# Irish-77/adapting-2D-ViTs-for-3D-point-cloud-understanding

Measured on NVIDIA B200. Metric: tokenized clouds/sec (FPS+kNN+embed), higher is better.
Workload: dtype bf16

## Files before the change

adapting-2d-vits-for-3d-point-cloud-understanding_b200/csrc/knn.cu:

```cuda
#include <stdlib.h>

#include "common.cuh"

namespace p3tok {

constexpr int KNN_WARPS = 8;
constexpr int KNN_CPW = 4;
constexpr int KNN_TILE = 2048;
constexpr uint64_t KNN_SENTINEL = 0xffffffffffffffffull;

__device__ __forceinline__ uint64_t shfl_xor_u64(uint64_t v, int m) {
  uint32_t lo = (uint32_t)v, hi = (uint32_t)(v >> 32);
  lo = __shfl_xor_sync(0xffffffffu, lo, m);
  hi = __shfl_xor_sync(0xffffffffu, hi, m);
  return ((uint64_t)hi << 32) | lo;
}
__device__ __forceinline__ uint64_t shfl_u64(uint64_t v, int src) {
  uint32_t lo = (uint32_t)v, hi = (uint32_t)(v >> 32);
  lo = __shfl_sync(0xffffffffu, lo, src);
  hi = __shfl_sync(0xffffffffu, hi, src);
  return ((uint64_t)hi << 32) | lo;
}
__device__ __forceinline__ uint64_t umin64(uint64_t a, uint64_t b) { return a < b ? a : b; }
__device__ __forceinline__ uint64_t umax64(uint64_t a, uint64_t b) { return a < b ? b : a; }
// ... 164 lines not shown
  if (g0 >= G) return;
#pragma unroll
  for (int c = 0; c < KNN_CPW; ++c) {
    if (qn[c] > 0) (void)merge_queue(c, L[c], qn[c]);
    const int g = g0 + c;
    if (g >= G) continue;
    const size_t o = ((size_t)b * G + g) * k;
#pragma unroll
    for (int j = 0; j < KPL; ++j) {
      const int r = j * 32 + lane;
      if (r < k) {
        const uint32_t id = (uint32_t)L[c][j];
        if (idx_is_i64) reinterpret_cast<int64_t*>(idx_out)[o + r] = (int64_t)id;
        else reinterpret_cast<int32_t*>(idx_out)[o + r] = (int32_t)id;
        if (dist_out) dist_out[o + r] = ord2f((uint32_t)(L[c][j] >> 32));
      }
    }
  }
}

template <int KPL>
static int knn_launch(const float* x, int B, int N, int pt_stride, const float* centres, int G, int k,
                      int mode, void* idx_out, int i64, float* dist_out, cudaStream_t s) {
  dim3 grid((unsigned)((G + KNN_WARPS * KNN_CPW - 1) / (KNN_WARPS * KNN_CPW)), (unsigned)B);
  if (mode == P3TOK_KNN_APF_SQ)
    knn_kernel<KPL, P3TOK_KNN_APF_SQ><<<grid, KNN_WARPS * 32, 0, s>>>(x, N, pt_stride, centres, G, k, idx_out, i64, dist_out);
  else
    knn_kernel<KPL, P3TOK_KNN_P4P_CDIST><<<grid, KNN_WARPS * 32, 0, s>>>(x, N, pt_stride, centres, G, k, idx_out, i64, dist_out);
  P3_LAUNCH_CHECK("knn_kernel");
  return P3TOK_OK;
}


#ifndef KNS_MIN_BLOCKS
#define KNS_MIN_BLOCKS 5
#endif
constexpr int KNS_MAX_N = 8192;
constexpr int KNS_MAX_SEG = 16;
constexpr int KNS_CELLS = 512;

struct KnsLayout {
  int64_t S, seg, nblk_seg;
  int64_t off_pts, off_ids, off_bb, off_lut, off_meta, total;
};
static KnsLayout kns_layout(int64_t B, int64_t N) {
  KnsLayout L;
  L.S = (N + KNS_MAX_N - 1) / KNS_MAX_N;
  L.seg = (N + L.S - 1) / L.S;
  L.nblk_seg = (L.seg + 31) / 32;
  const int64_t nblk = L.S * L.nblk_seg;
  int64_t o = 0;
  L.off_pts = o; o += B * nblk * 32 * 16;
  L.off_ids = o; o += B * nblk * 32 * 4;
  L.off_bb = o; o += B * nblk * 32;
  L.off_lut = o; o += B * L.S * (KNS_CELLS + 1) * 4;
  L.off_meta = o; o += B * L.S * 32;
  L.total = o + 256;
  return L;
}

__device__ __forceinline__ uint32_t kns_part1by2(uint32_t n) {
  n &= 0x000003ff;
  n = (n ^ (n << 16)) & 0xff0000ff;
  n = (n ^ (n << 8)) & 0x0300f00f;
  n = (n ^ (n << 4)) & 0x030c30c3;
  n = (n ^ (n << 2)) & 0x09249249;
// ... 311 lines not shown
                             const float* centres, int G, int64_t total, int k, int mode, void* idx_out, int i64, float* dist_out,
                             cudaStream_t s) {
  const unsigned grid = (unsigned)((total + KNN_WARPS - 1) / KNN_WARPS);
  static int bf = -1;
  if (bf < 0) { const char* e = getenv("P3TOK_KNN_BEST_FIRST"); bf = e ? atoi(e) : 1; }
  if (mode == P3TOK_KNN_APF_SQ)
    knn_sorted_kernel<KPL, P3TOK_KNN_APF_SQ><<<grid, KNN_WARPS * 32, 0, s>>>(pts, ids, bb, lut, meta, S, nblk, centres, G, total, k, idx_out, i64, dist_out, bf);
  else
    knn_sorted_kernel<KPL, P3TOK_KNN_P4P_CDIST><<<grid, KNN_WARPS * 32, 0, s>>>(pts, ids, bb, lut, meta, S, nblk, centres, G, total, k, idx_out, i64, dist_out, bf);
  P3_LAUNCH_CHECK("knn_sorted_kernel");
  return P3TOK_OK;
}

}

using namespace p3tok;

extern "C" int p3tok_knn(const float* x, int64_t B, int64_t N, int64_t pt_stride, const float* centres,
                         int64_t G, int64_t k, int mode, void* idx_out, int idx_dtype, float* dist_out,
                         void* stream) {
  P3_REQUIRE(B >= 0 && N > 0 && G >= 0 && pt_stride >= 3, P3TOK_ERR_INVALID, "knn: bad shape");
  P3_REQUIRE(mode == P3TOK_KNN_APF_SQ || mode == P3TOK_KNN_P4P_CDIST, P3TOK_ERR_INVALID, "knn: bad mode %d", mode);
  P3_REQUIRE(idx_dtype == P3TOK_I64 || idx_dtype == P3TOK_I32, P3TOK_ERR_INVALID, "knn: idx dtype must be i32/i64");
  P3_REQUIRE(k >= 1 && k <= N, P3TOK_ERR_INVALID, "knn: k=%lld out of range for N=%lld", (long long)k, (long long)N);
  P3_REQUIRE(k <= 128, P3TOK_ERR_UNSUPPORTED, "knn: k=%lld > 128", (long long)k);
  P3_REQUIRE(N < (1ll << 31) && B < 65536, P3TOK_ERR_UNSUPPORTED, "knn: N or B too large");
  if (B == 0 || G == 0) return P3TOK_OK;
  P3_REQUIRE(x && centres && idx_out, P3TOK_ERR_INVALID, "knn: null pointer");
  cudaStream_t s = as_stream(stream);
  const int i64 = idx_dtype == P3TOK_I64;
  if (k <= 32) return knn_launch<1>(x, (int)B, (int)N, (int)pt_stride, centres, (int)G, (int)k, mode, idx_out, i64, dist_out, s);
  if (k <= 64) return knn_launch<2>(x, (int)B, (int)N, (int)pt_stride, centres, (int)G, (int)k, mode, idx_out, i64, dist_out, s);
  return knn_launch<4>(x, (int)B, (int)N, (int)pt_stride, centres, (int)G, (int)k, mode, idx_out, i64, dist_out, s);
}

extern "C" int64_t p3tok_knn_workspace_bytes(int64_t B, int64_t N) {
  if (B < 0 || N <= 0 || N > (int64_t)KNS_MAX_N * KNS_MAX_SEG) return 0;
  return kns_layout(B, N).total;
}

struct KnsPtrs {
  float4* pts; int* ids; float* bb; int* lut; float* meta;
};
static KnsPtrs kns_ptrs(void* workspace, int64_t B, int64_t N) {
  const KnsLayout L = kns_layout(B, N);
  char* base = reinterpret_cast<char*>((reinterpret_cast<uintptr_t>(workspace) + 255) & ~(uintptr_t)255);
  KnsPtrs p;
  p.pts = reinterpret_cast<float4*>(base + L.off_pts);
  p.ids = reinterpret_cast<int*>(base + L.off_ids);
  p.bb = reinterpret_cast<float*>(base + L.off_bb);
  p.lut = reinterpret_cast<int*>(base + L.off_lut);
  p.meta = reinterpret_cast<float*>(base + L.off_meta);
  return p;
}

namespace p3tok {
int kns_workspace_views(const void* workspace, int64_t workspace_bytes, int64_t B, int64_t N, const float4** pts, const int** ids,
                        const float** bb) {
  P3_REQUIRE(N > 0 && N <= KNS_MAX_N && B >= 0, P3TOK_ERR_UNSUPPORTED, "sorted workspace: N=%lld outside (0, %d]", (long long)N, KNS_MAX_N);
  P3_REQUIRE(workspace_bytes >= kns_layout(B, N).total, P3TOK_ERR_WORKSPACE, "sorted workspace %lld < %lld bytes",
             (long long)workspace_bytes, (long long)kns_layout(B, N).total);
  const KnsPtrs w = kns_ptrs(const_cast<void*>(workspace), B, N);
  *pts = w.pts; *ids = w.ids; *bb = w.bb;
  return P3TOK_OK;
}
}
// ... 64 lines not shown
```

adapting-2d-vits-for-3d-point-cloud-understanding_b200/p3tok/_lib.py:

```python
from __future__ import annotations

import ctypes
import os
import re
from typing import List

_PKG = os.path.dirname(os.path.abspath(__file__))
LIB_PATH = os.environ.get("P3TOK_LIB") or os.path.join(_PKG, "libp3tok.so")
HEADER_PATH = os.path.join(os.path.dirname(os.path.dirname(_PKG)), "include", "p3tok.h")

OK, ERR_INVALID, ERR_UNSUPPORTED, ERR_CUDA, ERR_WORKSPACE = 0, 1, 2, 3, 4
KNN_APF_SQ, KNN_P4P_CDIST = 0, 1
F32, BF16, I32, I64, BF16X3 = 0, 1, 2, 3, 4
ROWS_APF, ROWS_P4P, ROWS_DIRECT = 0, 1, 2
EW_AXPBY, EW_MUL, EW_GELU, EW_GELU_BWD, EW_RELU, EW_RELU_BWD = 0, 1, 2, 3, 4, 5

_i32, _i64, _vp, _int = ctypes.c_int32, ctypes.c_int64, ctypes.c_void_p, ctypes.c_int


class MlpStruct(ctypes.Structure):
    _fields_ = [
        ("cin", _i32), ("n_pre", _i32), ("pre_dim", _i32 * 4), ("pre_relu", _i32 * 4),
        ("mid_dim", _i32), ("out_dim", _i32), ("out_relu", _i32), ("wdtype", _i32),
        ("w_pre", _vp * 4), ("b_pre", _vp * 4),
        ("w_mid_g", _vp), ("w_mid_f", _vp), ("b_mid", _vp), ("w_out", _vp), ("b_out", _vp),
    ]


class RowsStruct(ctypes.Structure):
    _fields_ = [
        ("kind", _i32), ("C", _i32), ("D", _i32), ("idx_dtype", _i32),
        ("B", _i64), ("N", _i64), ("G", _i64), ("k", _i64),
        ("x", _vp), ("feats", _vp), ("ctr_idx", _vp), ("knn_idx", _vp), ("perm", _vp),
    ]


class VitLayerStruct(ctypes.Structure):
    _fields_ = [(n, _vp) for n in ("qkv_w", "qkv_b", "proj_w", "proj_b", "fc1d_w", "fc1d_b", "fc2u_w", "fc2u_b")]


_f32 = ctypes.c_float

_SIGNATURES = {
    "p3tok_abi_version": (_int, []),
    "p3tok_last_error": (ctypes.c_char_p, []),
    "p3tok_kernel_launches": (_i64, []),
    "p3tok_fps": (_int, [_vp, _i64, _i64, _i64, _vp, _i64, _vp, _vp]),
    "p3tok_fps_sorted": (_int, [_vp, _i64, _i64, _i64, _vp, _i64, _vp, _vp]),
    "p3tok_fps_nd": (_int, [_vp, _i64, _i64, _i64, _i64, _vp, _i64, _vp, _vp, _vp]),
    "p3tok_square_distance": (_int, [_vp, _i64, _i64, _vp, _i64, _i64, _vp, _vp]),
    "p3tok_gather_points": (_int, [_vp, _i64, _i64, _i64, _vp, _i64, _vp, _vp]),
    "p3tok_knn": (_int, [_vp, _i64, _i64, _i64, _vp, _i64, _i64, _int, _vp, _int, _vp, _vp]),
    "p3tok_knn_workspace_bytes": (_i64, [_i64, _i64]),
    "p3tok_knn_sorted": (_int, [_vp, _i64, _i64, _i64, _vp, _i64, _i64, _int, _vp, _int, _vp, _vp, _i64, _vp]),
    "p3tok_knn_prepare": (_int, [_vp, _i64, _i64, _i64, _vp, _i64, _vp]),
    "p3tok_knn_query": (_int, [_vp, _i64, _i64, _i64, _vp, _i64, _i64, _int, _vp, _int, _vp, _vp]),
    "p3tok_morton_order": (_int, [_vp, _i64, _i64, _vp, _vp, _vp]),
    "p3tok_apf_group": (_int, [_vp, _i64, _i64, _i64, _vp, _vp, _vp, _i64, _i64, _vp, _vp, _vp]),
    "p3tok_group_gather": (_int, [_vp, _vp, _i64, _i64, _i64, _vp, _i64, _i64, _vp, _vp, _vp]),
    "p3tok_patch_embed_workspace_bytes": (_i64, [ctypes.POINTER(MlpStruct), _i64, _i64, _int]),
    "p3tok_patch_embed": (_int, [ctypes.POINTER(RowsStruct), ctypes.POINTER(MlpStruct), _int, _int, _vp, _i64, _vp, _vp]),
    "p3tok_linear_f32": (_int, [_vp, _i64, _i64, _vp, _i64, _vp, _vp, _i64, _int, _vp, _vp]),
    "p3tok_linear_x3_workspace_bytes": (_i64, [_i64, _i64, _i64]),
    "p3tok_linear_x3_f32": (_int, [_vp, _i64, _i64, _vp, _i64, _vp, _vp, _i64, _int, _vp, _vp, _i64, _vp]),
    "p3tok_linear_bf16": (_int, [_vp, _i64, _i64, _vp, _i64, _vp, _vp, _i64, _int, _vp, _vp, _vp, _vp]),
    "p3tok_token_head_f32": (_int, [_vp, _vp, _i64, _i64, _i64, _i64, _i64] + [_vp] * 12),
    "p3tok_group_max": (_int, [_vp, _i64, _i64, _i64, _vp, _vp]),
    "p3tok_linear_tn_f32": (_int, [_vp, _vp, _i64, _i64, _i64, _vp, _int, _vp]),
    "p3tok_colstats_f32": (_int, [_vp, _i64, _i64, _vp, _vp, _vp]),
    "p3tok_bn_act_f32": (_int, [_vp, _i64, _i64, _vp, _vp, _vp, _vp, _int, _vp, _vp]),
    "p3tok_bn_bwd_stats_f32": (_int, [_vp, _vp, _i64, _i64, _vp, _vp, _vp, _vp, _int, _vp, _vp, _vp]),
    "p3tok_bn_bwd_apply_f32": (_int, [_vp, _vp, _i64, _i64, _i64, _vp, _vp, _vp, _vp, _int, _vp, _vp, _vp, _vp]),
    "p3tok_group_max_arg_f32": (_int, [_vp, _i64, _i64, _i64, _vp, _vp, _vp]),
    "p3tok_group_max_bwd_f32": (_int, [_vp, _vp, _i64, _i64, _i64, _int, _vp, _vp]),
    "p3tok_group_sum_f32": (_int, [_vp, _i64, _i64, _i64, _vp, _vp]),
    "p3tok_scatter_rows_add_f32": (_int, [_vp, _vp, _i64, _i64, _i64, _i64, _i64, _vp, _vp, _vp]),
    "p3tok_build_rows_f32": (_int, [ctypes.POINTER(RowsStruct), _vp, _vp]),
    "p3tok_ln_fwd_f32": (_int, [_vp, _i64, _i64, _vp, _vp, _f32, _vp, _vp, _vp, _vp]),
    "p3tok_ln_bwd_f32": (_int, [_vp, _vp, _i64, _i64, _vp, _vp, _vp, _int, _vp, _vp]),
    "p3tok_ln_param_grad_f32": (_int, [_vp, _vp, _i64, _i64, _vp, _vp, _vp, _vp, _vp]),
    "p3tok_attn_fwd_f32": (_int, [_vp, _i64, _i64, _i64, _i64, _f32, _vp, _vp, _vp]),
    "p3tok_attn_bwd_f32": (_int, [_vp, _vp, _vp, _i64, _i64, _i64, _i64, _f32, _vp, _vp, _vp]),
    "p3tok_ew_f32": (_int, [_int, _vp, _vp, _f32, _f32, _i64, _i64, _vp, _vp]),
    "p3tok_apf_vit_workspace_bytes": (_i64, [_i64, _i64, _i64, _i64, _i64]),
    "p3tok_apf_vit_forward": (_int, [_vp, _i64, _i64, _i64, _i64, _i64, _i64, ctypes.POINTER(VitLayerStruct), _i64, _vp, _vp,
# ... 46 lines not shown
```

adapting-2d-vits-for-3d-point-cloud-understanding_b200/p3tok/modules.py:

```python
from __future__ import annotations

import math
from typing import List, Optional, Tuple

import torch
from torch import nn

from . import _lib, fold, ops, train
from .functional import _start


def _check_precision(p: str) -> bool:
    if p not in ("fp32", "bf16", "fp32tc"):
        raise ValueError(f"precision must be 'fp32', 'fp32tc' or 'bf16', got {p!r}")
    return p == "bf16"


def _check_token_dtype(token_dtype, precision: str) -> bool:
    if token_dtype in (None, torch.float32):
        return False
    if token_dtype != torch.bfloat16:
        raise ValueError(f"token_dtype must be torch.float32 or torch.bfloat16, got {token_dtype!r}")
    if precision != "bf16":
        raise ValueError("token_dtype=torch.bfloat16 needs precision='bf16'")
# ... 3 lines not shown
def _bn_eps(module: nn.Module):
    return {name: float(m.eps) for name, m in module.named_modules()
            if isinstance(m, (nn.BatchNorm1d, nn.BatchNorm2d))}


class _FoldedMixin:

    def _folded(self, build, device, bf16: bool) -> fold.PatchMLP:
        ver = tuple((t._version, t.data_ptr()) for t in list(self.parameters()) + list(self.buffers()))
        cache = self.__dict__.setdefault("_fold_cache", {})
        if cache.get("ver") != ver:
            cache.clear()
            cache["ver"] = ver
            cache["host"] = build()
        if getattr(self, "precision", None) == "fp32tc":
            return cache["host"].to_x3(device)
        return cache["host"].to(device, torch.bfloat16 if bf16 else torch.float32)

    def _require_eval(self):
        if self.training:
            raise RuntimeError(
                f"{type(self).__name__}: p3tok implements the eval-mode (folded BatchNorm) forward only; "
                "call .eval() first (training-mode batch statistics are out of scope, SURVEY.md 8f)")


class Group(nn.Module):

    def __init__(self, num_group: int, group_size: int):
        super().__init__()
        self.num_group = num_group
        self.group_size = group_size

    def indices(self, x: torch.Tensor, start_idx: Optional[torch.Tensor] = None):
        fps_idx, ws = ops.fps_with_knn_prepare(x, _start(x, start_idx), self.num_group)
        center = ops.gather_points(x, fps_idx)[..., :3].contiguous() if x.shape[-1] != 3 else ops.gather_points(x, fps_idx)
        knn_idx = ops.knn_query(x, ws, center, self.group_size, _lib.KNN_APF_SQ, False)
        perm = ops.morton_order(center)[0]
        return fps_idx, center, knn_idx, perm

    @staticmethod
    def _xyz_is_prefix_of(x: torch.Tensor, xyz: torch.Tensor) -> bool:
        return (xyz.shape[-1] == 3 and xyz.dtype == x.dtype and xyz.device == x.device and xyz.data_ptr() == x.data_ptr()
                and xyz.stride() == x.stride())

    def forward(self, x: torch.Tensor, xyz: torch.Tensor, start_idx: Optional[torch.Tensor] = None):
        if xyz.shape[:2] != x.shape[:2] or xyz.shape[-1] != 3:
            raise RuntimeError("Group.forward: xyz must be (B,N,3) with x's B and N")
        if x.dtype == torch.float32 and x.is_contiguous() and self._xyz_is_prefix_of(x, xyz):
            fps_idx, _, knn_idx, perm = self.indices(x, start_idx)
            return ops.apf_group(x, fps_idx, knn_idx, perm)
        x = x.float().contiguous()
        pts = xyz.float().contiguous()
        fps_idx, center, knn_idx, perm = self.indices(pts, start_idx)
        neigh, _ = ops.apf_group(x, fps_idx, knn_idx, perm)
        center = torch.gather(center, 1, perm.unsqueeze(-1).expand(-1, -1, 3))
        return neigh, center


class Encoder(nn.Module, _FoldedMixin):

    def __init__(self, encoder_channel: int, in_channel: int, precision: str = "fp32", token_dtype=None, sync_bn: bool = False):
        super().__init__()
        self.encoder_channel = encoder_channel
        self.precision = precision
        self.token_dtype = token_dtype
        self.sync_bn = sync_bn
        E = encoder_channel
# ... 78 lines not shown
            in_channels = W
            embed_dim *= 2
        self.out_channels = self.channel_list[-1]

    def folded(self, device) -> List[fold.PatchMLP]:
        bf16 = _check_precision(self.precision)
        ver = tuple((t._version, t.data_ptr()) for t in list(self.parameters()) + list(self.buffers()))
        cache = self.__dict__.setdefault("_fold_cache", {})
        if cache.get("ver") != ver:
            cache.clear()
            cache["ver"] = ver
            sd = self.state_dict()
            eps = _bn_eps(self)
            cache["host"] = [fold.fold_p3embed_stage(sd, s, eps) for s in range(len(self.convs))]
        if self.precision == "fp32tc":
            return [m.to_x3(device) for m in cache["host"]]
        return [m.to(device, torch.bfloat16 if bf16 else torch.float32) for m in cache["host"]]

    def forward(self, p: torch.Tensor, f: torch.Tensor, start_idx: Optional[List[torch.Tensor]] = None
                ) -> Tuple[List[torch.Tensor], List[torch.Tensor]]:
        if self.training:
            return self._forward_train(p, f, start_idx)
        bf16 = _check_precision(self.precision)
        B, N = int(p.shape[0]), int(p.shape[1])
        out_p, out_f = [p], [f]
        pts = p.float().contiguous()
        feat = f.float().transpose(1, 2).contiguous()
        folded = self.folded(p.device)
        bf16_last = _check_token_dtype(self.token_dtype, self.precision)
        for s, m in enumerate(folded):
            N = N // 4
            G = min(N, int(pts.shape[1]))
            st = None if start_idx is None else start_idx[s]
            cidx, ws = ops.fps_with_knn_prepare(pts, _start(pts, st, device_draw=True), G)
            ctr = ops.gather_points(pts, cidx)
            kidx = ops.knn_query(pts, ws, ctr, self.k, _lib.KNN_P4P_CDIST, True)
            tok = ops.patch_embed(_lib.ROWS_P4P, pts, feat, None, kidx, None, B * G, self.k, m.tensors(), m.meta(), bf16,
                                  bf16_last and s == len(folded) - 1, self.precision == "fp32tc")
            feat = tok.view(B, G, -1)
            pts = ctr
            out_p.append(ctr)
            out_f.append(feat.transpose(1, 2))
        return out_p, out_f


def _p3embed_forward_train(self, p, f, start_idx=None):
    B, N = int(p.shape[0]), int(p.shape[1])
    out_p, out_f = [p], [f]
    pts = p.float()
    feat = f.float().transpose(1, 2)
    for s, (conv1, conv2) in enumerate(self.convs):
        N = N // 4
        G = min(N, int(pts.shape[1]))
        st = None if start_idx is None else start_idx[s]
        with torch.no_grad():
            pd = pts.detach().contiguous()
            cidx, ws = ops.fps_with_knn_prepare(pd, _start(pd, st, device_draw=True), G)
            ctr_nd = ops.gather_points(pd, cidx)
            kidx = ops.knn_query(pd, ws, ctr_nd, self.k, _lib.KNN_P4P_CDIST, True)
        ctr = torch.gather(pts, 1, cidx.unsqueeze(-1).expand(-1, -1, 3))
        rows = train.GatherRowsFn.apply(pts.contiguous(), feat.contiguous(), kidx)
        tok = train.p3stage_train(conv1, conv2, rows, self.k, self.sync_bn)
        feat = tok.view(B, G, -1)
        pts = ctr
        out_p.append(ctr)
        out_f.append(feat.transpose(1, 2))
    return out_p, out_f


P3Embed._forward_train = _p3embed_forward_train


class PointViTTokens(nn.Module):

    def __init__(self, in_channels: int = 3, embed_dim: int = 384, k_neighbors: int = 16, precision: str = "fp32",
                 **p3embed_kwargs):
        super().__init__()
        self.num_features = self.embed_dim = embed_dim
        self.patch_embed = P3Embed(in_channels=in_channels, k=k_neighbors, precision=precision, **p3embed_kwargs)
        self.proj = nn.Linear(self.patch_embed.out_channels, embed_dim)
        self.pos_embed = nn.Sequential(nn.Linear(3, 128, bias=True), nn.GELU(), nn.Linear(128, embed_dim))
        self.cls_token = nn.Parameter(torch.zeros(1, 1, embed_dim))
        self.cls_pos = nn.Parameter(torch.zeros(1, 1, embed_dim))

    def forward(self, p: torch.Tensor, x: Optional[torch.Tensor] = None, start_idx: Optional[List[torch.Tensor]] = None):
        if x is None:
            x = p.transpose(1, 2)
        p_list, x_list = self.patch_embed(p, x, start_idx)
        tokens = x_list[-1].transpose(1, 2)
        if self.training or (torch.is_grad_enabled() and tokens.requires_grad):
# ... 9 lines not shown
```

adapting-2d-vits-for-3d-point-cloud-understanding_b200/p3tok/ops.py:

```python
from __future__ import annotations

import ctypes
import os
from typing import List, Optional, Sequence, Tuple

import torch

from . import _lib
from ._lib import check

_lib_handle = None


def _L():
    global _lib_handle
    if _lib_handle is None:
        _lib_handle = _lib.lib()
    return _lib_handle


def _stream() -> int:
    return torch.cuda.current_stream().cuda_stream


# ... 138 lines not shown
    B, S, N = int(c.shape[0]), int(c.shape[1]), int(d.shape[1])
    out = torch.empty((B, S, N), dtype=torch.float32, device=c.device)
    with torch.cuda.device(c.device), _timed("sqdist"):
        check(_L().p3tok_square_distance(c.data_ptr(), B, S, d.data_ptr(), N, stride, out.data_ptr(), _stream()),
              "square_distance")
    return out


@square_distance.register_fake
def _(src, dst):
    return src.new_empty((src.shape[0], src.shape[1], dst.shape[1]), dtype=torch.float32)


@torch.library.custom_op("p3tok::gather_points", mutates_args=(), device_types="cuda")
def gather_points(x: torch.Tensor, idx: torch.Tensor) -> torch.Tensor:
    _need_cuda("gather_points", x, idx)
    x = _f32c("gather_points", x)
    B, N, C = (int(v) for v in x.shape)
    flat = idx.to(torch.int64).reshape(B, -1).contiguous()
    S = int(flat.shape[1])
    out = torch.empty((B, S, C), dtype=torch.float32, device=x.device)
    with torch.cuda.device(x.device), _timed("gather"):
        check(_L().p3tok_gather_points(x.data_ptr(), B, N, C, flat.data_ptr(), S, out.data_ptr(), _stream()),
              "gather_points")
    return out.view(*idx.shape, C)


@gather_points.register_fake
def _(x, idx):
    return x.new_empty((*idx.shape, x.shape[-1]))


_KNN_SORTED = os.environ.get("P3TOK_KNN_SORTED", "1") != "0"
_OVERLAP = os.environ.get("P3TOK_OVERLAP", "auto")


@torch.library.custom_op("p3tok::knn", mutates_args=(), device_types="cuda")
def knn(x: torch.Tensor, centres: torch.Tensor, k: int, mode: int, int32_out: bool,
        return_dist: bool) -> Tuple[torch.Tensor, torch.Tensor]:
    _need_cuda("knn", x, centres)
    x = x if x.dtype == torch.float32 else x.float()
    x, stride = _point_stride(x)
    c = _f32c("knn", centres[..., :3])
    B, N = int(x.shape[0]), int(x.shape[1])
    if c.dim() != 3 or c.shape[0] != B:
        raise RuntimeError("p3tok::knn: centres must be (B,G,3)")
    G = int(c.shape[1])
    if k > N:
        raise RuntimeError(f"p3tok::knn: selected index k out of range (k={k} > N={N})")
    idx = torch.empty((B, G, k), dtype=torch.int32 if int32_out else torch.int64, device=x.device)
    dist = torch.empty((B, G, k) if return_dist else (0,), dtype=torch.float32, device=x.device)
    ws_bytes = int(_L().p3tok_knn_workspace_bytes(B, N)) if _KNN_SORTED and B * G > 0 else 0
    with torch.cuda.device(x.device), _timed("knn"):
        if ws_bytes > 0:
            ws = torch.empty(ws_bytes, dtype=torch.uint8, device=x.device)
            check(_L().p3tok_knn_sorted(x.data_ptr(), B, N, stride, c.data_ptr(), G, k, mode, idx.data_ptr(),
                                        _lib.I32 if int32_out else _lib.I64, dist.data_ptr() if return_dist else None,
                                        ws.data_ptr(), ws_bytes, _stream()), "knn_sorted")
        else:
            check(_L().p3tok_knn(x.data_ptr(), B, N, stride, c.data_ptr(), G, k, mode, idx.data_ptr(),
                                 _lib.I32 if int32_out else _lib.I64, dist.data_ptr() if return_dist else None,
                                 _stream()), "knn")
    return idx, dist


@knn.register_fake
def _(x, centres, k, mode, int32_out, return_dist):
    B, G = x.shape[0], centres.shape[1]
    return (x.new_empty((B, G, k), dtype=torch.int32 if int32_out else torch.int64),
            x.new_empty((B, G, k) if return_dist else (0,), dtype=torch.float32))


@torch.library.custom_op("p3tok::knn_prepare", mutates_args=(), device_types="cuda")
def knn_prepare(x: torch.Tensor) -> torch.Tensor:
    _need_cuda("knn_prepare", x)
    x_in = x
    x = x if x.dtype == torch.float32 else x.float()
    x, stride = _point_stride(x)
    B, N = int(x.shape[0]), int(x.shape[1])
    ws_bytes = int(_L().p3tok_knn_workspace_bytes(B, N)) if _KNN_SORTED and B > 0 else 0
    ws = torch.empty(max(ws_bytes, 0), dtype=torch.uint8, device=x.device)
    if ws_bytes > 0:
        with torch.cuda.device(x.device), _timed("knn"):
            check(_L().p3tok_knn_prepare(x.data_ptr(), B, N, stride, ws.data_ptr(), ws_bytes, _stream()), "knn_prepare")
        _ws_bind(ws, x_in)
    return ws


@knn_prepare.register_fake
def _(x):
    return x.new_empty((0,), dtype=torch.uint8)


@torch.library.custom_op("p3tok::knn_query", mutates_args=(), device_types="cuda")
def knn_query(x: torch.Tensor, ws: torch.Tensor, centres: torch.Tensor, k: int, mode: int, int32_out: bool) -> torch.Tensor:
    if ws.numel() == 0:
        return knn(x, centres, k, mode, int32_out, False)[0]
    _need_cuda("knn_query", x, ws, centres)
    _ws_check(ws, x)
    c = _f32c("knn_query", centres[..., :3])
    B, N, G = int(x.shape[0]), int(x.shape[1]), int(c.shape[1])
    if c.dim() != 3 or c.shape[0] != B:
        raise RuntimeError("p3tok::knn_query: centres must be (B,G,3)")
    if k > N:
        raise RuntimeError(f"p3tok::knn: selected index k out of range (k={k} > N={N})")
    idx = torch.empty((B, G, k), dtype=torch.int32 if int32_out else torch.int64, device=x.device)
    with torch.cuda.device(x.device), _timed("knn"):
        check(_L().p3tok_knn_query(ws.data_ptr(), int(ws.numel()), B, N, c.data_ptr(), G, k, mode, idx.data_ptr(),
                                   _lib.I32 if int32_out else _lib.I64, None, _stream()), "knn_query")
    return idx


@knn_query.register_fake
def _(x, ws, centres, k, mode, int32_out):
    return x.new_empty((x.shape[0], centres.shape[1], k), dtype=torch.int32 if int32_out else torch.int64)


_WS_OWNER = {}


def _ws_key(x: torch.Tensor):
    return (x.data_ptr(), tuple(x.shape), tuple(x.stride()), x._version)


def _ws_bind(ws: torch.Tensor, x: torch.Tensor) -> None:
    if len(_WS_OWNER) > 64:
        _WS_OWNER.clear()
    _WS_OWNER[ws.data_ptr()] = _ws_key(x)


def _ws_check(ws: torch.Tensor, x: torch.Tensor) -> None:
    owner = _WS_OWNER.get(ws.data_ptr())
    if owner is not None and owner != _ws_key(x):
        raise RuntimeError("p3tok::knn_query: this workspace was prepared from a different (or since modified) point tensor; "
                           "call knn_prepare(x) again")


@torch.library.custom_op("p3tok::fps_sorted", mutates_args=(), device_types="cuda")
def fps_sorted(x: torch.Tensor, ws: torch.Tensor, start_idx: torch.Tensor, npoint: int) -> torch.Tensor:
    _need_cuda("fps_sorted", x, ws, start_idx)
    _ws_check(ws, x)
    B, N = int(x.shape[0]), int(x.shape[1])
    start = start_idx.to(torch.int64).contiguous()
    if start.shape != (B,):
        raise RuntimeError(f"p3tok::fps: start_idx must have shape ({B},)")
    out = torch.empty((B, npoint), dtype=torch.int64, device=x.device)
    with torch.cuda.device(x.device), _timed("fps"):
        check(_L().p3tok_fps_sorted(ws.data_ptr(), int(ws.numel()), B, N, start.data_ptr(), npoint, out.data_ptr(), _stream()),
              "fps_sorted")
    return out


@fps_sorted.register_fake
def _(x, ws, start_idx, npoint):
    return x.new_empty((x.shape[0], npoint), dtype=torch.int64)


def fps_with_knn_prepare(x: torch.Tensor, start_idx: torch.Tensor, npoint: int) -> Tuple[torch.Tensor, torch.Tensor]:
    _need_cuda("fps_with_knn_prepare", x)
    if _use_culled_fps(int(x.shape[0]), int(x.shape[1]), npoint):
        ws = knn_prepare(x)
        return fps_sorted(x, ws, start_idx, npoint), ws
    if _OVERLAP == "0" or (_OVERLAP != "1" and 2 * int(x.shape[0]) > _sm_count(x.device)):
        return fps(x, start_idx, npoint), knn_prepare(x)
    cur = torch.cuda.current_stream(x.device)
    side = _side_stream(x.device)
    side.wait_stream(cur)
    with torch.cuda.stream(side):
        ws = knn_prepare(x)
    idx = fps(x, start_idx, npoint)
    cur.wait_stream(side)
    ws.record_stream(cur)
    return idx, ws


_SIDE = {}
_SMS = {}


def _sm_count(device) -> int:
    key = device.index if device.index is not None else torch.cuda.current_device()
    if key not in _SMS:
        _SMS[key] = torch.cuda.get_device_properties(key).multi_processor_count
    return _SMS[key]


def _side_stream(device) -> torch.cuda.Stream:
    key = (device.index if device.index is not None else torch.cuda.current_device())
    s = _SIDE.get(key)
    if s is None:
        s = _SIDE[key] = torch.cuda.Stream(device=device)
    return s
# ... 420 lines not shown
```

include/p3tok.h:

```cpp
#ifndef P3TOK_H_
#define P3TOK_H_

#include <stdint.h>

#ifdef __cplusplus
extern "C" {
#endif

#define P3TOK_ABI_VERSION 2

#if defined(__GNUC__)
#define P3TOK_API __attribute__((visibility("default")))
#else
#define P3TOK_API
#endif

enum p3tok_status {
  P3TOK_OK = 0,
  P3TOK_ERR_INVALID = 1,
  P3TOK_ERR_UNSUPPORTED = 2,
  P3TOK_ERR_CUDA = 3,
  P3TOK_ERR_WORKSPACE = 4
};

enum p3tok_knn_mode {
  P3TOK_KNN_APF_SQ = 0,
  P3TOK_KNN_P4P_CDIST = 1
};

enum p3tok_dtype { P3TOK_F32 = 0, P3TOK_BF16 = 1, P3TOK_I32 = 2, P3TOK_I64 = 3,
                   P3TOK_BF16X3 = 4  };

P3TOK_API int p3tok_abi_version(void);
P3TOK_API const char* p3tok_last_error(void);
P3TOK_API int64_t p3tok_kernel_launches(void);

P3TOK_API int p3tok_fps(const float* x, int64_t B, int64_t N, int64_t pt_stride, const int64_t* start_idx,
              int64_t G, int64_t* out_idx, void* stream);

P3TOK_API int p3tok_fps_sorted(const void* workspace, int64_t workspace_bytes, int64_t B, int64_t N,
                     const int64_t* start_idx, int64_t G, int64_t* out_idx, void* stream);

P3TOK_API int p3tok_fps_nd(const float* x, int64_t B, int64_t N, int64_t D, int64_t pt_stride, const int64_t* start_idx,
                 int64_t G, int64_t* out_idx, float* min_dist_ws, void* stream);

P3TOK_API int p3tok_gather_points(const float* x, int64_t B, int64_t N, int64_t C, const int64_t* idx,
                        int64_t S, float* out, void* stream);

P3TOK_API int p3tok_knn(const float* x, int64_t B, int64_t N, int64_t pt_stride, const float* centres,
              int64_t G, int64_t k, int mode, void* idx_out, int idx_dtype, float* dist_out,
              void* stream);

P3TOK_API int64_t p3tok_knn_workspace_bytes(int64_t B, int64_t N);
P3TOK_API int p3tok_knn_sorted(const float* x, int64_t B, int64_t N, int64_t pt_stride, const float* centres,
                     int64_t G, int64_t k, int mode, void* idx_out, int idx_dtype, float* dist_out,
                     void* workspace, int64_t workspace_bytes, void* stream);

P3TOK_API int p3tok_knn_prepare(const float* x, int64_t B, int64_t N, int64_t pt_stride, void* workspace,
                      int64_t workspace_bytes, void* stream);
P3TOK_API int p3tok_knn_query(const void* workspace, int64_t workspace_bytes, int64_t B, int64_t N, const float* centres,
                    int64_t G, int64_t k, int mode, void* idx_out, int idx_dtype, float* dist_out, void* stream);

P3TOK_API int p3tok_square_distance(const float* src, int64_t B, int64_t S, const float* dst, int64_t N,
                          int64_t dst_stride, float* out, void* stream);

P3TOK_API int p3tok_morton_order(const float* centres, int64_t B, int64_t G, int64_t* perm,
                       int64_t* codes_out, void* stream);

P3TOK_API int p3tok_apf_group(const float* x, int64_t B, int64_t N, int64_t C, const int64_t* fps_idx,
                    const int64_t* knn_idx, const int64_t* perm, int64_t G, int64_t k,
                    float* neigh, float* center, void* stream);

P3TOK_API int p3tok_group_gather(const float* pnts, const float* feats, int64_t B, int64_t N, int64_t D,
                       const int32_t* idx, int64_t G, int64_t k, float* grouped_pnts,
                       float* grouped_feats, void* stream);

typedef struct p3tok_mlp {
  int32_t cin;
  int32_t n_pre;
  int32_t pre_dim[4];
  int32_t pre_relu[4];
  int32_t mid_dim;
  int32_t out_dim;
  int32_t out_relu;
// ... 112 lines not shown
```

Measured before the change: 153,800.

## Add shared-memory small-cloud kNN kernel and skip sorted workspace prepare

```diff
diff --git a/adapting-2d-vits-for-3d-point-cloud-understanding_b200/csrc/knn.cu b/adapting-2d-vits-for-3d-point-cloud-understanding_b200/csrc/knn.cu
--- a/adapting-2d-vits-for-3d-point-cloud-understanding_b200/csrc/knn.cu
+++ b/adapting-2d-vits-for-3d-point-cloud-understanding_b200/csrc/knn.cu
@@ -220,6 +220,183 @@
 }
 
 
+constexpr int KNN_SMALL_MAX_N = KNN_TILE;
+constexpr int KNN_SMALL_MAX_K = 32;
+
+__device__ __forceinline__ uint64_t cx_keep(uint64_t v, int j, bool keep_min) {
+  const uint64_t o = shfl_xor_u64(v, j);
+  return ((o < v) == keep_min) ? o : v;
+}
+__device__ __forceinline__ float cx_keep(float v, int j, bool keep_min) {
+  const float o = __shfl_xor_sync(0xffffffffu, v, j);
+  return keep_min ? fminf(v, o) : fmaxf(v, o);
+}
+template <typename T>
+__device__ __forceinline__ T sort32_asc(T v, int lane) {
+#pragma unroll
+  for (int k = 2; k <= 32; k <<= 1) {
+#pragma unroll
+    for (int j = k >> 1; j > 0; j >>= 1) v = cx_keep(v, j, ((lane & k) == 0) == ((lane & j) == 0));
+  }
+  return v;
+}
+template <typename T>
+__device__ __forceinline__ T bitonic32_asc(T v, int lane) {
+#pragma unroll
+  for (int j = 16; j > 0; j >>= 1) v = cx_keep(v, j, (lane & j) == 0);
+  return v;
+}
+
+template <int MODE>
+__global__ void __launch_bounds__(KNN_WARPS * 32, 4)
+knn_small_kernel(const float* __restrict__ x, int N, int pt_stride, const float* __restrict__ centres, int G, int k,
+                 void* __restrict__ idx_out, int idx_is_i64, float* __restrict__ dist_out) {
+  extern __shared__ float4 cloud[];
+  __shared__ uint64_t queue[KNN_WARPS * KNN_CPW][64];
+  const float INF = __int_as_float(0x7f800000);
+  constexpr float FMAX = 3.40282347e38f;
+  constexpr float SQ_MARGIN = 1.0000002384185791f;
+
+  const int t = threadIdx.x, lane = t & 31, warp = t >> 5;
+  const int b = blockIdx.y;
+  const int g0 = (blockIdx.x * KNN_WARPS + warp) * KNN_CPW;
+  const float* P = x + (size_t)b * N * pt_stride;
+#pragma unroll 4
+  for (int i = t; i < N; i += KNN_WARPS * 32) {
+    const float* pp = P + (size_t)i * pt_stride;
+    const float px = pp[0], py = pp[1], pz = pp[2];
+    cloud[i] = make_float4(px, py, pz, sq3(px, py, pz));
+  }
+  __syncthreads();
+  if (g0 >= G) return;
+
+  float c0[KNN_CPW], c1[KNN_CPW], c2[KNN_CPW], cn[KNN_CPW];
+#pragma unroll
+  for (int c = 0; c < KNN_CPW; ++c) {
+    const int g = min(g0 + c, G - 1);
+    const float* cp = centres + ((size_t)b * G + g) * 3;
+    const float cx = cp[0], cy = cp[1], cz = cp[2];
+    cn[c] = sq3(cx, cy, cz);
+    if (MODE == P3TOK_KNN_APF_SQ) {
+      c0[c] = cx; c1[c] = cy; c2[c] = cz;
+    } else {
+      c0[c] = __fmul_rn(-2.f, cx); c1[c] = __fmul_rn(-2.f, cy); c2[c] = __fmul_rn(-2.f, cz);
+    }
+  }
+  auto pre = [&](int c, const float4 p) -> float {
+    if (MODE == P3TOK_KNN_APF_SQ) {
+      const float dot = __fmaf_rn(c2[c], p.z, __fmaf_rn(c1[c], p.y, __fmul_rn(c0[c], p.x)));
+      return __fadd_rn(__fadd_rn(__fmul_rn(-2.f, dot), cn[c]), p.w);
+    } else {
+      float tt = __fmul_rn(c0[c], p.x);
+      tt = __fmaf_rn(c1[c], p.y, tt);
+      tt = __fmaf_rn(c2[c], p.z, tt);
+      tt = __fadd_rn(tt, cn[c]);
+      return __fadd_rn(tt, p.w);
+    }
+  };
+
+  float m1[KNN_CPW], m2[KNN_CPW];
+#pragma unroll
+  for (int c = 0; c < KNN_CPW; ++c) m1[c] = m2[c] = INF;
+#pragma unroll 2
+  for (int i = lane; i < N; i += 32) {
+    const float4 p = cloud[i];
+#pragma unroll
+    for (int c = 0; c < KNN_CPW; ++c) {
+      float d = pre(c, p);
+      d = d < INF ? d : INF;
+      m2[c] = fminf(m2[c], fmaxf(m1[c], d));
+      m1[c] = fminf(m1[c], d);
+    }
+  }
+  float thr[KNN_CPW];
+  float thr_d[KNN_CPW];
+#pragma unroll
+  for (int c = 0; c < KNN_CPW; ++c) {
+    const float a = sort32_asc(m1[c], lane), bb = sort32_asc(m2[c], lane);
+    const float lo = bitonic32_asc(fminf(a, __shfl_sync(0xffffffffu, bb, 31 - lane)), lane);
+    const float tau = __shfl_sync(0xffffffffu, lo, k - 1);
+    if (MODE == P3TOK_KNN_APF_SQ) {
+      thr[c] = tau < INF ? tau : FMAX;
+      thr_d[c] = thr[c];
+    } else {
+      const float td = tau < INF ? __fadd_rn(__fsqrt_rn(fmaxf(tau, 0.f)), 0.f) : FMAX;
+      thr_d[c] = td;
+      thr[c] = __fmul_ru(__fmul_ru(td, td), SQ_MARGIN);
+    }
+  }
+
+  uint64_t L[KNN_CPW];
+  int qn[KNN_CPW];
+#pragma unroll
+  for (int c = 0; c < KNN_CPW; ++c) { L[c] = KNN_SENTINEL; qn[c] = 0; }
+  auto merge_queue = [&](int c, int cnt) {
+    const uint64_t* q = queue[warp * KNN_CPW + c];
+    uint64_t v = (lane < cnt) ? q[lane] : KNN_SENTINEL;
+    if (MODE == P3TOK_KNN_P4P_CDIST && v != KNN_SENTINEL) {
+      const float d = __fadd_rn(__fsqrt_rn(fmaxf(ord2f((uint32_t)(v >> 32)), 0.f)), 0.f);
+      v = d < INF ? (((uint64_t)f2ord(d) << 32) | (uint32_t)v) : KNN_SENTINEL;
+    }
+    v = sort32_asc(v, lane);
+    L[c] = bitonic32_asc(umin64(L[c], shfl_u64(v, 31 - lane)), lane);
+    const uint32_t ko = (uint32_t)(shfl_u64(L[c], k - 1) >> 32);
+    if (ko != 0xffffffffu) {
+      const float kd = ord2f(ko);
+      if (MODE == P3TOK_KNN_APF_SQ) {
+        thr[c] = fminf(thr[c], kd);
+      } else {
+        thr_d[c] = fminf(thr_d[c], kd);
+        thr[c] = __fmul_ru(__fmul_ru(thr_d[c], thr_d[c]), SQ_MARGIN);
+      }
+    }
+  };
+
+  for (int i0 = 0; i0 < N; i0 += 32) {
+    const int i = i0 + lane;
+    const bool valid = i < N;
+    const float4 p = cloud[valid ? i : 0];
+    float dc[KNN_CPW];
+    bool pc[KNN_CPW];
+    bool any = false;
+#pragma unroll
+    for (int c = 0; c < KNN_CPW; ++c) {
+      dc[c] = pre(c, p);
+      pc[c] = valid && (dc[c] <= thr[c]);
+      any = any || pc[c];
+    }
+    if (!__any_sync(0xffffffffu, any)) continue;
+#pragma unroll
+    for (int c = 0; c < KNN_CPW; ++c) {
+      const uint32_t ball = __ballot_sync(0xffffffffu, pc[c]);
+      if (ball == 0) continue;
+      const float d = MODE == P3TOK_KNN_APF_SQ ? __fadd_rn(dc[c], 0.f) : dc[c];
+      uint64_t* q = queue[warp * KNN_CPW + c];
+      if (pc[c]) q[qn[c] + __popc(ball & ((1u << lane) - 1u))] = ((uint64_t)f2ord(d) << 32) | (uint32_t)i;
+      qn[c] += __popc(ball);
+      __syncwarp();
+      if (qn[c] >= 32) {
+        merge_queue(c, 32);
+        __syncwarp();
+        if (lane + 32 < qn[c]) q[lane] = q[lane + 32];
+        qn[c] -= 32;
+        __syncwarp();
+      }
+    }
+  }
+#pragma unroll
+  for (int c = 0; c < KNN_CPW; ++c) {
+    if (qn[c] > 0) merge_queue(c, qn[c]);
+    const int g = g0 + c;
+    if (g >= G || lane >= k) continue;
+    const size_t o = ((size_t)b * G + g) * k + lane;
+    const uint32_t id = (uint32_t)L[c];
+    if (idx_is_i64) reinterpret_cast<int64_t*>(idx_out)[o] = (int64_t)id;
+    else reinterpret_cast<int32_t*>(idx_out)[o] = (int32_t)id;
+    if (dist_out) dist_out[o] = ord2f((uint32_t)(L[c] >> 32));
+  }
+}
+
 #ifndef KNS_MIN_BLOCKS
 #define KNS_MIN_BLOCKS 5
 #endif
@@ -597,6 +774,33 @@
   if (k <= 32) return knn_launch<1>(x, (int)B, (int)N, (int)pt_stride, centres, (int)G, (int)k, mode, idx_out, i64, dist_out, s);
   if (k <= 64) return knn_launch<2>(x, (int)B, (int)N, (int)pt_stride, centres, (int)G, (int)k, mode, idx_out, i64, dist_out, s);
   return knn_launch<4>(x, (int)B, (int)N, (int)pt_stride, centres, (int)G, (int)k, mode, idx_out, i64, dist_out, s);
+}
+
+extern "C" int p3tok_knn_small(const float* x, int64_t B, int64_t N, int64_t pt_stride, const float* centres,
+                               int64_t G, int64_t k, int mode, void* idx_out, int idx_dtype, float* dist_out,
+                               void* stream) {
+  P3_REQUIRE(B >= 0 && N > 0 && G >= 0 && pt_stride >= 3, P3TOK_ERR_INVALID, "knn_small: bad shape");
+  P3_REQUIRE(mode == P3TOK_KNN_APF_SQ || mode == P3TOK_KNN_P4P_CDIST, P3TOK_ERR_INVALID, "knn_small: bad mode %d", mode);
+  P3_REQUIRE(idx_dtype == P3TOK_I64 || idx_dtype == P3TOK_I32, P3TOK_ERR_INVALID, "knn_small: idx dtype must be i32/i64");
+  P3_REQUIRE(k >= 1 && k <= N, P3TOK_ERR_INVALID, "knn_small: k=%lld out of range for N=%lld", (long long)k, (long long)N);
+  P3_REQUIRE(N <= KNN_SMALL_MAX_N && k <= KNN_SMALL_MAX_K, P3TOK_ERR_UNSUPPORTED,
+             "knn_small: N=%lld, k=%lld outside N <= %d, k <= %d (use p3tok_knn)", (long long)N, (long long)k, KNN_SMALL_MAX_N,
+             KNN_SMALL_MAX_K);
+  P3_REQUIRE(B < 65536, P3TOK_ERR_UNSUPPORTED, "knn_small: B too large");
+  if (B == 0 || G == 0) return P3TOK_OK;
+  P3_REQUIRE(x && centres && idx_out, P3TOK_ERR_INVALID, "knn_small: null pointer");
+  const dim3 grid((unsigned)((G + KNN_WARPS * KNN_CPW - 1) / (KNN_WARPS * KNN_CPW)), (unsigned)B);
+  const size_t smem = (size_t)N * sizeof(float4);
+  const int i64 = idx_dtype == P3TOK_I64;
+  cudaStream_t s = as_stream(stream);
+  if (mode == P3TOK_KNN_APF_SQ)
+    knn_small_kernel<P3TOK_KNN_APF_SQ><<<grid, KNN_WARPS * 32, smem, s>>>(x, (int)N, (int)pt_stride, centres, (int)G, (int)k,
+                                                                          idx_out, i64, dist_out);
+  else
+    knn_small_kernel<P3TOK_KNN_P4P_CDIST><<<grid, KNN_WARPS * 32, smem, s>>>(x, (int)N, (int)pt_stride, centres, (int)G, (int)k,
+                                                                             idx_out, i64, dist_out);
+  P3_LAUNCH_CHECK("knn_small_kernel");
+  return P3TOK_OK;
 }
 
 extern "C" int64_t p3tok_knn_workspace_bytes(int64_t B, int64_t N) {
diff --git a/adapting-2d-vits-for-3d-point-cloud-understanding_b200/p3tok/_lib.py b/adapting-2d-vits-for-3d-point-cloud-understanding_b200/p3tok/_lib.py
--- a/adapting-2d-vits-for-3d-point-cloud-understanding_b200/p3tok/_lib.py
+++ b/adapting-2d-vits-for-3d-point-cloud-understanding_b200/p3tok/_lib.py
@@ -51,6 +51,7 @@
     "p3tok_square_distance": (_int, [_vp, _i64, _i64, _vp, _i64, _i64, _vp, _vp]),
     "p3tok_gather_points": (_int, [_vp, _i64, _i64, _i64, _vp, _i64, _vp, _vp]),
     "p3tok_knn": (_int, [_vp, _i64, _i64, _i64, _vp, _i64, _i64, _int, _vp, _int, _vp, _vp]),
+    "p3tok_knn_small": (_int, [_vp, _i64, _i64, _i64, _vp, _i64, _i64, _int, _vp, _int, _vp, _vp]),
     "p3tok_knn_workspace_bytes": (_i64, [_i64, _i64]),
     "p3tok_knn_sorted": (_int, [_vp, _i64, _i64, _i64, _vp, _i64, _i64, _int, _vp, _int, _vp, _vp, _i64, _vp]),
     "p3tok_knn_prepare": (_int, [_vp, _i64, _i64, _i64, _vp, _i64, _vp]),
diff --git a/adapting-2d-vits-for-3d-point-cloud-understanding_b200/p3tok/modules.py b/adapting-2d-vits-for-3d-point-cloud-understanding_b200/p3tok/modules.py
--- a/adapting-2d-vits-for-3d-point-cloud-understanding_b200/p3tok/modules.py
+++ b/adapting-2d-vits-for-3d-point-cloud-understanding_b200/p3tok/modules.py
@@ -59,7 +59,7 @@
         self.group_size = group_size
 
     def indices(self, x: torch.Tensor, start_idx: Optional[torch.Tensor] = None):
-        fps_idx, ws = ops.fps_with_knn_prepare(x, _start(x, start_idx), self.num_group)
+        fps_idx, ws = ops.fps_with_knn_prepare(x, _start(x, start_idx), self.num_group, self.group_size)
         center = ops.gather_points(x, fps_idx)[..., :3].contiguous() if x.shape[-1] != 3 else ops.gather_points(x, fps_idx)
         knn_idx = ops.knn_query(x, ws, center, self.group_size, _lib.KNN_APF_SQ, False)
         perm = ops.morton_order(center)[0]
@@ -204,7 +204,7 @@
             N = N // 4
             G = min(N, int(pts.shape[1]))
             st = None if start_idx is None else start_idx[s]
-            cidx, ws = ops.fps_with_knn_prepare(pts, _start(pts, st, device_draw=True), G)
+            cidx, ws = ops.fps_with_knn_prepare(pts, _start(pts, st, device_draw=True), G, self.k)
             ctr = ops.gather_points(pts, cidx)
             kidx = ops.knn_query(pts, ws, ctr, self.k, _lib.KNN_P4P_CDIST, True)
             tok = ops.patch_embed(_lib.ROWS_P4P, pts, feat, None, kidx, None, B * G, self.k, m.tensors(), m.meta(), bf16,
@@ -227,7 +227,7 @@
         st = None if start_idx is None else start_idx[s]
         with torch.no_grad():
             pd = pts.detach().contiguous()
-            cidx, ws = ops.fps_with_knn_prepare(pd, _start(pd, st, device_draw=True), G)
+            cidx, ws = ops.fps_with_knn_prepare(pd, _start(pd, st, device_draw=True), G, self.k)
             ctr_nd = ops.gather_points(pd, cidx)
             kidx = ops.knn_query(pd, ws, ctr_nd, self.k, _lib.KNN_P4P_CDIST, True)
         ctr = torch.gather(pts, 1, cidx.unsqueeze(-1).expand(-1, -1, 3))
diff --git a/adapting-2d-vits-for-3d-point-cloud-understanding_b200/p3tok/ops.py b/adapting-2d-vits-for-3d-point-cloud-understanding_b200/p3tok/ops.py
--- a/adapting-2d-vits-for-3d-point-cloud-understanding_b200/p3tok/ops.py
+++ b/adapting-2d-vits-for-3d-point-cloud-understanding_b200/p3tok/ops.py
@@ -194,6 +194,12 @@
 
 
 _KNN_SORTED = os.environ.get("P3TOK_KNN_SORTED", "1") != "0"
+_KNN_SMALL = os.environ.get("P3TOK_KNN_SMALL", "1") != "0"
+_KNN_SMALL_MAX_N, _KNN_SMALL_MAX_K = 2048, 32
+
+
+def knn_small_applies(N: int, k: int) -> bool:
+    return _KNN_SORTED and _KNN_SMALL and 1 <= k <= N <= _KNN_SMALL_MAX_N and k <= _KNN_SMALL_MAX_K
 _OVERLAP = os.environ.get("P3TOK_OVERLAP", "auto")
 
 
@@ -212,9 +218,14 @@
         raise RuntimeError(f"p3tok::knn: selected index k out of range (k={k} > N={N})")
     idx = torch.empty((B, G, k), dtype=torch.int32 if int32_out else torch.int64, device=x.device)
     dist = torch.empty((B, G, k) if return_dist else (0,), dtype=torch.float32, device=x.device)
-    ws_bytes = int(_L().p3tok_knn_workspace_bytes(B, N)) if _KNN_SORTED and B * G > 0 else 0
+    small = knn_small_applies(N, k)
+    ws_bytes = int(_L().p3tok_knn_workspace_bytes(B, N)) if _KNN_SORTED and not small and B * G > 0 else 0
     with torch.cuda.device(x.device), _timed("knn"):
-        if ws_bytes > 0:
+        if small:
+            check(_L().p3tok_knn_small(x.data_ptr(), B, N, stride, c.data_ptr(), G, k, mode, idx.data_ptr(),
+                                       _lib.I32 if int32_out else _lib.I64, dist.data_ptr() if return_dist else None,
+                                       _stream()), "knn_small")
+        elif ws_bytes > 0:
             ws = torch.empty(ws_bytes, dtype=torch.uint8, device=x.device)
             check(_L().p3tok_knn_sorted(x.data_ptr(), B, N, stride, c.data_ptr(), G, k, mode, idx.data_ptr(),
                                         _lib.I32 if int32_out else _lib.I64, dist.data_ptr() if return_dist else None,
@@ -266,6 +277,8 @@
         raise RuntimeError("p3tok::knn_query: centres must be (B,G,3)")
     if k > N:
         raise RuntimeError(f"p3tok::knn: selected index k out of range (k={k} > N={N})")
+    if knn_small_applies(N, k):
+        return knn(x, centres, k, mode, int32_out, False)[0]
     idx = torch.empty((B, G, k), dtype=torch.int32 if int32_out else torch.int64, device=x.device)
     with torch.cuda.device(x.device), _timed("knn"):
         check(_L().p3tok_knn_query(ws.data_ptr(), int(ws.numel()), B, N, c.data_ptr(), G, k, mode, idx.data_ptr(),
@@ -318,8 +331,11 @@
     return x.new_empty((x.shape[0], npoint), dtype=torch.int64)
 
 
-def fps_with_knn_prepare(x: torch.Tensor, start_idx: torch.Tensor, npoint: int) -> Tuple[torch.Tensor, torch.Tensor]:
+def fps_with_knn_prepare(x: torch.Tensor, start_idx: torch.Tensor, npoint: int,
+                         k: Optional[int] = None) -> Tuple[torch.Tensor, torch.Tensor]:
     _need_cuda("fps_with_knn_prepare", x)
+    if k is not None and knn_small_applies(int(x.shape[1]), k) and not _use_culled_fps(int(x.shape[0]), int(x.shape[1]), npoint):
+        return fps(x, start_idx, npoint), x.new_empty((0,), dtype=torch.uint8)
     if _use_culled_fps(int(x.shape[0]), int(x.shape[1]), npoint):
         ws = knn_prepare(x)
         return fps_sorted(x, ws, start_idx, npoint), ws
diff --git a/include/p3tok.h b/include/p3tok.h
--- a/include/p3tok.h
+++ b/include/p3tok.h
@@ -50,6 +50,10 @@
 P3TOK_API int p3tok_knn(const float* x, int64_t B, int64_t N, int64_t pt_stride, const float* centres,
               int64_t G, int64_t k, int mode, void* idx_out, int idx_dtype, float* dist_out,
               void* stream);
+
+P3TOK_API int p3tok_knn_small(const float* x, int64_t B, int64_t N, int64_t pt_stride, const float* centres,
+                    int64_t G, int64_t k, int mode, void* idx_out, int idx_dtype, float* dist_out,
+                    void* stream);
 
 P3TOK_API int64_t p3tok_knn_workspace_bytes(int64_t B, int64_t N);
 P3TOK_API int p3tok_knn_sorted(const float* x, int64_t B, int64_t N, int64_t pt_stride, const float* centres,
diff --git a/profiles/knn_small_time.py b/profiles/knn_small_time.py
--- /dev/null
+++ b/profiles/knn_small_time.py
@@ -0,0 +1,84 @@
+import argparse
+import json
+import os
+import sys
+
+ROOT = os.path.dirname(os.path.dirname(os.path.abspath(__file__)))
+sys.path.insert(0, os.path.join(ROOT, "adapting-2d-vits-for-3d-point-cloud-understanding_b200"))
+sys.dont_write_bytecode = True
+
+import torch
+
+from p3tok import _lib, ops, synth
+
+SHAPES = [
+    ("c2", 128, 2048, 128, 32, _lib.KNN_APF_SQ, False),
+    ("c5_stage0", 4096, 1024, 256, 32, _lib.KNN_P4P_CDIST, True),
+    ("c5_stage1", 4096, 256, 64, 32, _lib.KNN_P4P_CDIST, True),
+    ("c3_stage1", 256, 2048, 512, 32, _lib.KNN_P4P_CDIST, True),
+]
+
+
+def main():
+    ap = argparse.ArgumentParser()
+    ap.add_argument("--reps", type=int, default=20)
+    ap.add_argument("--rounds", type=int, default=5)
+    ap.add_argument("--out", help="also append the JSON lines to this file")
+    args = ap.parse_args()
+    assert torch.cuda.is_available(), "needs a CUDA device"
+    dev = torch.device("cuda:0")
+    L = ops._L()
+    props = torch.cuda.get_device_properties(dev)
+    lines = []
+    for name, B, N, G, k, mode, i32 in SHAPES:
+        x = torch.from_numpy(synth.make_cloud("uniform", B, N, 11, 3)).to(dev)
+        st = torch.from_numpy(synth.start_indices(B, N, 11)).to(dev)
+        ctr = ops.gather_points(x, ops.fps(x, st, G)).contiguous()
+        dt = _lib.I32 if i32 else _lib.I64
+        s = torch.cuda.current_stream().cuda_stream
+        nbytes = int(L.p3tok_knn_workspace_bytes(B, N))
+        ws = torch.empty(nbytes, dtype=torch.uint8, device=dev)
+        outs = {a: torch.empty((B, G, k), dtype=torch.int32 if i32 else torch.int64, device=dev)
+                for a in ("sorted", "small", "sweep")}
+
+        def run(arm):
+            o = outs[arm].data_ptr()
+            if arm == "sorted":
+                _lib.check(L.p3tok_knn_prepare(x.data_ptr(), B, N, 3, ws.data_ptr(), nbytes, s), "knn_prepare")
+                _lib.check(L.p3tok_knn_query(ws.data_ptr(), nbytes, B, N, ctr.data_ptr(), G, k, mode, o, dt, None, s), "knn_query")
+            elif arm == "small":
+                _lib.check(L.p3tok_knn_small(x.data_ptr(), B, N, 3, ctr.data_ptr(), G, k, mode, o, dt, None, s), "knn_small")
+            else:
+                _lib.check(L.p3tok_knn(x.data_ptr(), B, N, 3, ctr.data_ptr(), G, k, mode, o, dt, None, s), "knn")
+
+        for arm in outs:
+            for _ in range(3):
+                run(arm)
+        torch.cuda.synchronize()
+        same = torch.equal(outs["sorted"], outs["sweep"]) and torch.equal(outs["small"], outs["sweep"])
+        ms = {a: [] for a in outs}
+        for _ in range(args.rounds):
+            for arm in outs:
+                e0, e1 = torch.cuda.Event(enable_timing=True), torch.cuda.Event(enable_timing=True)
+                e0.record()
+                for _ in range(args.reps):
+                    run(arm)
+                e1.record()
+                torch.cuda.synchronize()
+                ms[arm].append(e0.elapsed_time(e1) / args.reps)
+        med = {a: sorted(v)[len(v) // 2] for a, v in ms.items()}
+        line = {"shape": name, "B": B, "N": N, "G": G, "k": k, "mode": "apf_sq" if mode == _lib.KNN_APF_SQ else "p4p_cdist",
+                "identical_indices": same, "ms_median": {a: round(v, 4) for a, v in med.items()},
+                "ms_spread": {a: [round(min(v), 4), round(max(v), 4)] for a, v in ms.items()},
+                "speedup_small_vs_sorted": round(med["sorted"] / med["small"], 3),
+                "gpu": props.name, "reps_per_round": args.reps, "rounds": args.rounds}
+        print(json.dumps(line), flush=True)
+        lines.append(line)
+    if args.out:
+        with open(args.out, "a") as f:
+            for line in lines:
+                f.write(json.dumps(line) + "\n")
+
+
+if __name__ == "__main__":
+    main()
```

Result: faster. 158,000 (median of 6 runs) (+2.7%).
